# MPEGGroup/mpeg-pcc-tmc2

Hardware: AMD Instinct MI355X
Metric: encoder patch+image-gen frames/sec, longdress_vox10 32-frame GOF (higher is better)
Workload: dtype int32/f64

## Files before the change

### mpeg-pcc-tmc2_amd/csrc/attributes.hip

```cpp
#include <algorithm>
#include <cmath>

#include "color_transfer.h"
#include "internal.h"
#include "wave.h"
#include "patch_border_filter.h"

namespace tmc2 {
namespace {

__device__ __forceinline__ void toCanvasB( const PlaceDev& p, int u, int v, int& x, int& y ) {
  if ( p.orient == 0 ) {
    x = u + p.u0 * 16;
    y = v + p.v0 * 16;
  } else {
    x = v + p.u0 * 16;
    y = u + p.v0 * 16;
  }
}

__device__ __forceinline__ int normalCoord( const PlaceDev& p, int depth ) {
  return p.mode == 0 ? depth + p.d1 : max( 0, p.d1 - depth );
}

// ... 115 lines not shown
  reinterpret_cast<uchar4*>( outRgb4 )[t] = combinedColor( reinterpret_cast<const uchar4*>( fwdRgb4 )[t], c );
}

__device__ __forceinline__ CtColor ctColorOf( const uint8_t* __restrict__ rgb4, uint32_t i ) {
  const uchar4 c = reinterpret_cast<const uchar4*>( rgb4 )[i];
  return CtColor{c.x, c.y, c.z};
}
__device__ __forceinline__ void ctStore( uint8_t* __restrict__ rgb4, uint32_t i, const CtColor& c ) {
  reinterpret_cast<uchar4*>( rgb4 )[i] = make_uchar4( uint8_t( c.c0 ), uint8_t( c.c1 ), uint8_t( c.c2 ), 0 );
}
__global__ __launch_bounds__( 256 ) void forwardColorRulesKernel( const uint32_t* __restrict__ idx, const uint32_t* __restrict__ dist, int stride,
                                                                   const uint32_t* __restrict__ easy, const uint8_t* __restrict__ srcRgb4,
                                                                   uint32_t m, CtRules p, uint8_t* __restrict__ fwdRgb4 ) {
  const uint32_t t = blockIdx.x * blockDim.x + threadIdx.x;
  if ( t >= m ) return;
  if ( easy && easy[t] != 0xFFFFFFFFu ) {
    reinterpret_cast<uchar4*>( fwdRgb4 )[t] = reinterpret_cast<const uchar4*>( srcRgb4 )[easy[t]];
    return;
  }
  const uint32_t* id = idx + size_t( t ) * stride;
  const uint32_t* ds = dist + size_t( t ) * stride;
  ctStore( fwdRgb4, t, ctForward( p, p.kFwd, [ds]( int i ) { return ds[i]; }, [id, srcRgb4]( int i ) { return ctColorOf( srcRgb4, id[i] ); } ) );
}

template <bool FILL>
__global__ __launch_bounds__( 256 ) void backwardVoteRulesKernel( const uint32_t* __restrict__ idx, const uint32_t* __restrict__ dist, int stride,
                                                                   uint32_t n, int kBwd, double geoBwd, uint32_t* __restrict__ count,
                                                                   const uint32_t* __restrict__ offset, uint2* __restrict__ entries ) {
  const uint32_t s = blockIdx.x * blockDim.x + threadIdx.x;
  if ( s >= n ) return;
  for ( int r = 0; r < kBwd; ++r ) {
    const uint32_t d = dist[size_t( s ) * stride + r];
    if ( !( double( d ) <= geoBwd ) ) continue;
    const uint32_t t = idx[size_t( s ) * stride + r], slot = atomicAdd( &count[t], 1u );
    if ( FILL ) entries[offset[t] + slot] = make_uint2( d, s * uint32_t( kBwd ) + uint32_t( r ) );
  }
}

__global__ __launch_bounds__( 256 ) void combineColorRulesKernel( const uint32_t* __restrict__ count, const uint32_t* __restrict__ offset,
                                                                   uint2* __restrict__ entries, const uint8_t* __restrict__ srcRgb4,
                                                                   const uint8_t* __restrict__ fwdRgb4, uint32_t m, CtRules p, double rTarget,
                                                                   double rSource, uint8_t* __restrict__ outRgb4, uint32_t* __restrict__ error ) {
  const uint32_t t = blockIdx.x * blockDim.x + threadIdx.x;
  if ( t >= m ) return;
  const int     n   = int( count[t] );
  const CtColor fwd = ctColorOf( fwdRgb4, t );
  if ( n == 0 || p.lossless ) {
    ctStore( outRgb4, t, fwd );
    return;
  }
  uint2* e = entries + offset[t];
  if ( !orderCandidates( e, n ) ) *error = 1;
  const uint32_t kBwd = uint32_t( p.kBwd );
  ctStore( outRgb4, t,
           ctBackward( p, n, [e]( int i ) { return e[i].x; }, [e, srcRgb4, kBwd]( int i ) { return ctColorOf( srcRgb4, e[i].y / kBwd ); }, fwd,
                       rTarget, rSource ) );
}

__global__ __launch_bounds__( 256 ) void attributeScatterKernel( const uint8_t* __restrict__ rgb4,
                                                                  const uint32_t* __restrict__ pointToPixel, uint32_t m,
                                                                  int W, int H, uint8_t* __restrict__ attr ) {
  const uint32_t i = blockIdx.x * blockDim.x + threadIdx.x;
  if ( i >= m ) return;
  const uint32_t pp = pointToPixel[i];
  const size_t   px = size_t( pixelY( pp ) ) * W + pixelX( pp ), plane = size_t( W ) * H;
  const uchar4   c  = reinterpret_cast<const uchar4*>( rgb4 )[i];
  const bool     layer1 = pixelLayer( pp ), hasD1 = pixelHasD1( pp );
  if ( !layer1 ) {
    attr[px] = c.x, attr[plane + px] = c.y, attr[2 * plane + px] = c.z;
    if ( !hasD1 ) attr[3 * plane + px] = c.x, attr[4 * plane + px] = c.y, attr[5 * plane + px] = c.z;
  } else {
    attr[3 * plane + px] = c.x, attr[4 * plane + px] = c.y, attr[5 * plane + px] = c.z;
  }
}

__global__ __launch_bounds__( 256 ) void upsampleOccupancyKernel( const uint8_t* __restrict__ occVideo, int W, int H, int prec,
                                                                   uint8_t* __restrict__ occ ) {
  const size_t c = size_t( blockIdx.x ) * blockDim.x + threadIdx.x;
  if ( c >= size_t( W ) * H ) return;
  occ[c] = occVideo[size_t( ( c / W ) / prec ) * ( W / prec ) + ( c % W ) / prec];
}

__device__ __forceinline__ int mean4w( int p1, int w1, int p2, int w2, int p3, int w3, int p4, int w4 ) {
  return ( p1 * w1 + p2 * w2 + p3 * w3 + p4 * w4 ) / ( w1 + w2 + w3 + w4 );
}

__device__ __forceinline__ void pushPullMipPixel( int i, const uint8_t* img, const uint8_t* occ, int W, int H, uint8_t* mip,
                                                  uint8_t* mipOcc, int w, int h, int p0 = 0, int p1 = 6 ) {
  const int  x = i % w, y = i / w, X = 2 * x, Y = 2 * y;
  const bool i2 = X + 1 < W, i3 = Y + 1 < H;
  const int  w1 = occ[size_t( Y ) * W + X] ? 255 : 0;
  const int  w2 = ( i2 && occ[size_t( Y ) * W + X + 1] ) ? 255 : 0;
  const int  w3 = ( i3 && occ[size_t( Y + 1 ) * W + X] ) ? 255 : 0;
  const int  w4 = ( i2 && i3 && occ[size_t( Y + 1 ) * W + X + 1] ) ? 255 : 0;
  const bool any = ( w1 + w2 + w3 + w4 ) > 0;
  mipOcc[i]      = any ? 1 : 0;
  for ( int p = p0; p < p1; ++p ) {
    const uint8_t* s = img + size_t( p ) * W * H;
    uint8_t        v = 0;
    if ( any ) {
      const int v1 = s[size_t( Y ) * W + X], v2 = i2 ? s[size_t( Y ) * W + X + 1] : 0;
      const int v3 = i3 ? s[size_t( Y + 1 ) * W + X] : 0, v4 = ( i2 && i3 ) ? s[size_t( Y + 1 ) * W + X + 1] : 0;
      v            = uint8_t( mean4w( v1, w1, v2, w2, v3, w3, v4, w4 ) );
    }
    mip[size_t( p ) * w * h + i] = v;
  }
}
__global__ __launch_bounds__( 256 ) void pushPullMipKernel( const uint8_t* __restrict__ img, const uint8_t* __restrict__ occ, int W,
                                                             int H, uint8_t* __restrict__ mip, uint8_t* __restrict__ mipOcc, int w,
                                                             int h ) {
  const int i = blockIdx.x * blockDim.x + threadIdx.x;
  if ( i < w * h ) pushPullMipPixel( i, img, occ, W, H, mip, mipOcc, w, h );
}

__device__ __forceinline__ void pushPullFillPixel( int i, uint8_t* img, const uint8_t* occ, int W, int H, const uint8_t* mip, int w,
                                                   int h, int p0 = 0, int p1 = 6 ) {
  if ( occ[i] ) return;
  const int  X = i % W, Y = i / W, x = X >> 1, y = Y >> 1;
  const int  dx = ( X & 1 ) ? 1 : -1, dy = ( Y & 1 ) ? 1 : -1;
  const bool hx = dx < 0 ? x > 0 : x < w - 1, hy = dy < 0 ? y > 0 : y < h - 1;
  for ( int p = p0; p < p1; ++p ) {
    const uint8_t* m  = mip + size_t( p ) * w * h;
    const int      v  = m[size_t( y ) * w + x];
    const int      vx = hx ? m[size_t( y ) * w + x + dx] : 0;
    const int      vy = hy ? m[size_t( y + dy ) * w + x] : 0;
    const int      vd = ( hx && hy ) ? m[size_t( y + dy ) * w + x + dx] : 0;
    img[size_t( p ) * W * H + i] = uint8_t( mean4w( v, 144, vx, hx ? 48 : 0, vy, hy ? 48 : 0, vd, ( hx && hy ) ? 16 : 0 ) );
  }
}
__global__ __launch_bounds__( 256 ) void pushPullFillKernel( uint8_t* __restrict__ img, const uint8_t* __restrict__ occ, int W, int H,
                                                              const uint8_t* __restrict__ mip, int w, int h ) {
  const int i = blockIdx.x * blockDim.x + threadIdx.x;
  if ( i < W * H ) pushPullFillPixel( i, img, occ, W, H, mip, w, h );
}

__device__ __forceinline__ void pushPullBlurPixel( int i, const uint8_t* src, uint8_t* dst, const uint8_t* occ, int W, int H, int p0 = 0,
                                                   int p1 = 6 ) {
  if ( occ[i] ) return;
  const int x = i % W, y = i / W;
  const int x1 = x > 0 ? x - 1 : x, y1 = y > 0 ? y - 1 : y, x2 = x < W - 1 ? x + 1 : x, y2 = y < H - 1 ? y + 1 : y;
  for ( int p = p0; p < p1; ++p ) {
    const uint8_t* s   = src + size_t( p ) * W * H;
    const int      sum = s[size_t( y1 ) * W + x1] + s[size_t( y1 ) * W + x2] + s[size_t( y2 ) * W + x1] + s[size_t( y2 ) * W + x2] +
                    s[size_t( y ) * W + x1] + s[size_t( y ) * W + x2] + s[size_t( y1 ) * W + x] + s[size_t( y2 ) * W + x];
    dst[size_t( p ) * W * H + i] = uint8_t( ( sum + 4 ) >> 3 );
  }
}
__global__ __launch_bounds__( 256 ) void pushPullBlurKernel( const uint8_t* __restrict__ src, uint8_t* __restrict__ dst,
                                                              const uint8_t* __restrict__ occ, int W, int H ) {
  const int i = blockIdx.x * blockDim.x + threadIdx.x;
  if ( i < W * H ) pushPullBlurPixel( i, src, dst, occ, W, H );
}

constexpr int kPushPullTile = 96, kPushPullSpan = 128, kPushPullMaxIters = ( kPushPullSpan - kPushPullTile ) / 2;
__global__ __launch_bounds__( 1024 ) void pushPullFillBlurKernel( uint8_t* __restrict__ img, const uint8_t* __restrict__ occ, int W,
                                                                   int H, const uint8_t* __restrict__ mip, int w, int h, int iters,
                                                                   int tilesX ) {
  __shared__ uint8_t sOcc[kPushPullSpan * kPushPullSpan];
  __shared__ uint8_t sBuf[2][kPushPullSpan * kPushPullSpan];
  const int      X0 = ( blockIdx.x % tilesX ) * kPushPullTile, Y0 = ( blockIdx.x / tilesX ) * kPushPullTile;
  const int      RX0 = max( X0 - iters, 0 ), RY0 = max( Y0 - iters, 0 );
  const int      RW = min( X0 + kPushPullTile + iters, W ) - RX0, RH = min( Y0 + kPushPullTile + iters, H ) - RY0;
  uint8_t*       plane = img + size_t( blockIdx.y ) * W * H;
  const uint8_t* m     = mip + size_t( blockIdx.y ) * w * h;
  for ( int i = threadIdx.x; i < kPushPullSpan * RH; i += 1024 ) {
    const int rx = i & ( kPushPullSpan - 1 ), ry = i >> 7;
    if ( rx >= RW ) continue;
    const int     X = RX0 + rx, Y = RY0 + ry;
    const size_t  g = size_t( Y ) * W + X;
    const uint8_t o = occ[g];
    uint8_t       v;
    if ( o ) {
      v = plane[g];
    } else {
      const int  x = X >> 1, y = Y >> 1, dx = ( X & 1 ) ? 1 : -1, dy = ( Y & 1 ) ? 1 : -1;
      const bool hx = dx < 0 ? x > 0 : x < w - 1, hy = dy < 0 ? y > 0 : y < h - 1;
      const int  c  = m[size_t( y ) * w + x];
      const int  vx = hx ? m[size_t( y ) * w + x + dx] : 0;
      const int  vy = hy ? m[size_t( y + dy ) * w + x] : 0;
      const int  vd = ( hx && hy ) ? m[size_t( y + dy ) * w + x + dx] : 0;
      v             = uint8_t( mean4w( c, 144, vx, hx ? 48 : 0, vy, hy ? 48 : 0, vd, ( hx && hy ) ? 16 : 0 ) );
    }
    sOcc[i]    = o;
    sBuf[0][i] = v;
    sBuf[1][i] = v;
  }
  __syncthreads();
  int cur = 0;
  for ( int it = 0; it < iters; ++it ) {
    const uint8_t* src = sBuf[cur];
    uint8_t*       dst = sBuf[cur ^ 1];
    for ( int i = threadIdx.x; i < kPushPullSpan * RH; i += 1024 ) {
      const int rx = i & ( kPushPullSpan - 1 ), ry = i >> 7;
      if ( rx >= RW || sOcc[i] ) continue;
      const int l = rx > 0 ? -1 : 0, r = rx < RW - 1 ? 1 : 0;
      const int u = ry > 0 ? -kPushPullSpan : 0, d = ry < RH - 1 ? kPushPullSpan : 0;
      const int sum = src[i + u + l] + src[i + u + r] + src[i + d + l] + src[i + d + r] + src[i + l] + src[i + r] + src[i + u] +
                      src[i + d];
      dst[i] = uint8_t( ( sum + 4 ) >> 3 );
    }
    __syncthreads();
    cur ^= 1;
  }
  const uint8_t* res = sBuf[cur];
  for ( int i = threadIdx.x; i < kPushPullSpan * RH; i += 1024 ) {
    const int rx = i & ( kPushPullSpan - 1 ), ry = i >> 7;
    const int X = RX0 + rx, Y = RY0 + ry;
    if ( rx >= RW || sOcc[i] || X < X0 || X >= X0 + kPushPullTile || Y < Y0 || Y >= Y0 + kPushPullTile ) continue;
    plane[size_t( Y ) * W + X] = res[i];
  }
}

constexpr int kPushPullSmall  = 160 * 160;
constexpr int kPushPullLevels = 16;
struct PushPullLevels {
  int      count;
  int      first;
  int      w[kPushPullLevels], h[kPushPullLevels];
  uint8_t *img[kPushPullLevels], *tmp[kPushPullLevels], *occ[kPushPullLevels];
};
__global__ __launch_bounds__( 1024 ) void pushPullCoarseLevelsKernel( PushPullLevels L ) {
  const int p0 = int( blockIdx.x ), p1 = p0 + 1;
  for ( int l = L.first + 1; l < L.count; ++l ) {
    const int cnt = L.w[l] * L.h[l];
    for ( int i = threadIdx.x; i < cnt; i += blockDim.x )
      pushPullMipPixel( i, L.img[l - 1], L.occ[l - 1], L.w[l - 1], L.h[l - 1], L.img[l], L.occ[l], L.w[l], L.h[l], p0, p1 );
    __syncthreads();
  }
  int iters = 4;
  for ( int l = L.count - 1; l > L.first; --l ) {
    const int fw = L.w[l - 1], fh = L.h[l - 1], cnt = fw * fh;
    uint8_t * img = L.img[l - 1], *tmp = L.tmp[l - 1];
    const uint8_t* occ = L.occ[l - 1];
    for ( int i = threadIdx.x; i < cnt; i += blockDim.x ) pushPullFillPixel( i, img, occ, fw, fh, L.img[l], L.w[l], L.h[l], p0, p1 );
    __syncthreads();
    for ( int i = threadIdx.x; i < cnt; i += blockDim.x ) tmp[size_t( p0 ) * cnt + i] = img[size_t( p0 ) * cnt + i];
    __syncthreads();
    uint8_t *src = img, *dst = tmp;
    for ( int it = 0; it < iters; ++it ) {
      for ( int i = threadIdx.x; i < cnt; i += blockDim.x ) pushPullBlurPixel( i, src, dst, occ, fw, fh, p0, p1 );
      __syncthreads();
      uint8_t* t = src;
      src        = dst;
      dst        = t;
    }
    if ( src != img ) {
      L.img[l - 1] = src;
      L.tmp[l - 1] = img;
    }
    iters = min( iters + 1, 16 );
  }
}

__global__ __launch_bounds__( 256 ) void attributeGroupDilateKernel( const uint8_t* __restrict__ occ, int W, int H,
                                                                      uint8_t* __restrict__ attr ) {
  const size_t c = size_t( blockIdx.x ) * blockDim.x + threadIdx.x, plane = size_t( W ) * H;
  if ( c >= plane || occ[c] ) return;
#pragma unroll
  for ( int k = 0; k < 3; ++k ) {
    const uint32_t a = attr[k * plane + c], b = attr[( 3 + k ) * plane + c];
    const uint8_t  v = uint8_t( ( a + b + 1 ) >> 1 );
    attr[k * plane + c] = attr[( 3 + k ) * plane + c] = v;
  }
}

}

static int transferColorsRules( tmc2_ctx* ctx, const TreeDev& srcTree, const Pt* d_srcPts, const uint8_t* d_srcRgb4, uint32_t n,
                                const TreeDev& tgtTree, const Pt* d_tgtPts, uint32_t M, uint8_t* d_outRgb4, uint32_t* d_error,
                                const CtRules& p ) {
  hipStream_t      s = ctx->stream;
  const dim3       blk( 256 );
  const int        wf = knnWidth( p.kFwd ), wb = knnWidth( p.kBwd );
  DevBuf<uint32_t> d_idxF, d_distF, d_easyF, d_idxB, d_distB, d_count, d_offset, d_cursor;
  DevBuf<uint2>    d_entries;
  DevBuf<uint8_t>  d_fwd;
  TMC2_TRY( d_idxF.alloc( size_t( M ) * wf ) );
  TMC2_TRY( d_distF.alloc( size_t( M ) * wf ) );
  TMC2_TRY( d_idxB.alloc( size_t( n ) * wb ) );
  TMC2_TRY( d_distB.alloc( size_t( n ) * wb ) );
  TMC2_TRY( d_count.alloc( M ) );
  TMC2_TRY( d_offset.alloc( M ) );
  TMC2_TRY( d_cursor.alloc( M ) );
  TMC2_TRY( d_entries.alloc( size_t( n ) * p.kBwd ) );
  TMC2_TRY( d_fwd.alloc( size_t( M ) * 4 ) );
  if ( p.skipFwd ) {
    TMC2_TRY( d_easyF.alloc( M ) );
    TMC2_TRY( launchKnnSplit( ctx, srcTree, d_tgtPts, M, wf, d_easyF.p, d_idxF.p, d_distF.p, "knn_recon_in_source", false, p.kFwd ) );
  } else {
    TMC2_TRY( launchKnnTree( ctx, srcTree, d_tgtPts, M, wf, d_idxF.p, d_distF.p, "knn_recon_in_source", p.kFwd ) );
  }
  if ( p.kBwd == 1 )
    TMC2_TRY( launchKnnSplit( ctx, tgtTree, d_srcPts, n, 1, d_idxB.p, d_idxB.p, d_distB.p, "knn_source_in_recon" ) );
  else
    TMC2_TRY( launchKnnTree( ctx, tgtTree, d_srcPts, n, wb, d_idxB.p, d_distB.p, "knn_source_in_recon", p.kBwd ) );
  StageScope stage( ctx, "transfer_colors" );
  TMC2_TRY( fillRegions( ctx, {{d_count.p, size_t( M ) * 4, 0}, {d_cursor.p, size_t( M ) * 4, 0}, {d_error, 4, 0}} ) );
  const dim3 grdM( ( M + 255 ) / 256 ), grdN( ( n + 255 ) / 256 );
  hipLaunchKernelGGL( forwardColorRulesKernel, grdM, blk, 0, s, d_idxF.p, d_distF.p, wf, p.skipFwd ? d_easyF.p : (const uint32_t*)nullptr,
                      d_srcRgb4, M, p, d_fwd.p );
  hipLaunchKernelGGL( backwardVoteRulesKernel<false>, grdN, blk, 0, s, d_idxB.p, d_distB.p, wb, n, p.kBwd, p.geoBwd, d_count.p, d_offset.p,
                      d_entries.p );
  TMC2_TRY( exclusiveScanU32( ctx, d_count.p, d_offset.p, M, nullptr ) );
  hipLaunchKernelGGL( backwardVoteRulesKernel<true>, grdN, blk, 0, s, d_idxB.p, d_distB.p, wb, n, p.kBwd, p.geoBwd, d_cursor.p, d_offset.p,
                      d_entries.p );
  hipLaunchKernelGGL( combineColorRulesKernel, grdM, blk, 0, s, d_count.p, d_offset.p, d_entries.p, d_srcRgb4, d_fwd.p, M, p,
                      1.0 / double( M ), 1.0 / double( n ), d_outRgb4, d_error );
  TMC2_HIP( hipGetLastError() );
  return TMC2_OK;
}

int transferColorsDevice( tmc2_ctx* ctx, const TreeDev& srcTree, const Pt* d_srcPts, const uint8_t* d_srcRgb4, uint32_t n,
                          const TreeDev& tgtTree, const Pt* d_tgtPts, uint32_t M, uint8_t* d_outRgb4, uint32_t* d_error,
                          const tmc2_color_transfer_params* params = nullptr ) {
  const auto forced = ctxOption( ctx, "COLOR_TRANSFER_RULES" );
  if ( params && ( !ctIsDefault( *params ) || ( forced && ( *forced )[0] == '1' ) ) )
    return transferColorsRules( ctx, srcTree, d_srcPts, d_srcRgb4, n, tgtTree, d_tgtPts, M, d_outRgb4, d_error, ctRules( *params ) );
  hipStream_t      s = ctx->stream;
  const dim3       blk( 256 );
  DevBuf<uint32_t> d_idx8, d_dist8, d_idx1, d_dist1, d_count, d_offset, d_cursor;
  DevBuf<uint2>    d_entries;
  DevBuf<uint8_t>  d_fwd;
  TMC2_TRY( d_idx8.alloc( size_t( M ) * 8 ) );
  TMC2_TRY( d_dist8.alloc( size_t( M ) * 8 ) );
  TMC2_TRY( d_idx1.alloc( n ) );
  TMC2_TRY( d_dist1.alloc( n ) );
  TMC2_TRY( d_count.alloc( M ) );
  TMC2_TRY( d_offset.alloc( M ) );
  TMC2_TRY( d_cursor.alloc( M ) );
  TMC2_TRY( d_entries.alloc( n ) );
  TMC2_TRY( d_fwd.alloc( size_t( M ) * 4 ) );
  DevBuf<uint32_t> d_easy8;
  TMC2_TRY( d_easy8.alloc( M ) );
  TMC2_TRY( launchKnnSplit( ctx, srcTree, d_tgtPts, M, 8, d_easy8.p, d_idx8.p, d_dist8.p, "knn8_recon_in_source" ) );
  TMC2_TRY( launchKnnSplit( ctx, tgtTree, d_srcPts, n, 1, d_idx1.p, d_idx1.p, d_dist1.p, "knn1_source_in_recon" ) );
  StageScope stage( ctx, "transfer_colors" );
  TMC2_TRY( fillRegions( ctx, {{d_count.p, size_t( M ) * 4, 0}, {d_cursor.p, size_t( M ) * 4, 0}, {d_error, 4, 0}} ) );
  const dim3 grdM( ( M + 255 ) / 256 ), grdN( ( n + 255 ) / 256 );
  hipLaunchKernelGGL( forwardColorKernel, grdM, blk, 0, s, d_idx8.p, d_dist8.p, d_easy8.p, d_srcRgb4, M, d_fwd.p );
  hipLaunchKernelGGL( backwardVoteKernel<false>, grdN, blk, 0, s, d_idx1.p, d_dist1.p, n, d_count.p, d_offset.p, d_entries.p );
  TMC2_TRY( exclusiveScanU32( ctx, d_count.p, d_offset.p, M, nullptr ) );
  hipLaunchKernelGGL( backwardVoteKernel<true>, grdN, blk, 0, s, d_idx1.p, d_dist1.p, n, d_cursor.p, d_offset.p, d_entries.p );
  hipLaunchKernelGGL( combineColorKernel, grdM, blk, 0, s, d_count.p, d_offset.p, d_entries.p, d_srcRgb4, d_fwd.p, M,
                      d_outRgb4, d_error );
  TMC2_HIP( hipGetLastError() );
  return TMC2_OK;
}

int reconstructPointCloud( tmc2_frame* f, const PbfParams* pbfParams ) {
  if ( !f->haveGeometryImages ) {
    setError( "generatePointCloud: geometry images missing" );
    return TMC2_E_STATE;
  }
  if ( pbfParams ) {
    if ( const char* what = pbfRefusal( f->occPrecision, *pbfParams, long( f->patches.size() ) ) ) {
      setError( "generatePointCloud (patch border filtering): unsupported %s", what );
      return TMC2_E_UNSUPPORTED;
    }
  }
  const bool keepAttributeImages = f->haveAttributeImages && ( pbfParams || f->havePbf );
  f->canvasesChanged();
  f->haveAttributeImages = keepAttributeImages;
  if ( pbfParams ) TMC2_TRY( patchBorderFilterDevice( f, *pbfParams ) );
  PbfMapsDev pbf;
  if ( pbfParams ) pbf = PbfMapsDev{f->d_pbfOffset.p, f->pbfOcc, f->pbfFlag, f->pbfBorderWidth, nullptr};
  tmc2_ctx*    ctx = f->ctx;
  hipStream_t  s   = ctx->stream;
  const int    W = f->canvasW, H = f->canvasH, prec = f->occPrecision;
  const dim3   blk( 256 );
  const uint32_t tiles = f->tileCount;
  StageScope       stage( ctx, "reconstruct" );
  DevBuf<uint32_t> d_tileCount, d_tileOffset, d_small;
  TMC2_TRY( d_tileCount.alloc( std::max( tiles, 1u ) ) );
  TMC2_TRY( d_tileOffset.alloc( std::max( tiles, 1u ) ) );
  TMC2_TRY( d_small.alloc( 8 ) );
  uint32_t M = 0;
  if ( tiles ) {
    if ( pbfParams )
      hipLaunchKernelGGL( ( reconTileKernel<false, true> ), dim3( tiles ), blk, 0, s, f->d_place.p, f->d_tilePatch.p, f->d_occVideo.p,
                          f->d_blockToPatch.p, f->d_geo.p, W, H, prec, d_tileCount.p, (const uint32_t*)nullptr, (Pt*)nullptr,
                          (uint32_t*)nullptr, pbf );
    else
      hipLaunchKernelGGL( reconTileKernel<false>, dim3( tiles ), blk, 0, s, f->d_place.p, f->d_tilePatch.p, f->d_occVideo.p,
                          f->d_blockToPatch.p, f->d_geo.p, W, H, prec, d_tileCount.p, (const uint32_t*)nullptr, (Pt*)nullptr,
                          (uint32_t*)nullptr, PbfMapsDev() );
    volatile uint32_t* answer = ctx->answerLine( tmc2_ctx::kAnswerRecon );
    TMC2_TRY( exclusiveScanU32( ctx, d_tileCount.p, d_tileOffset.p, tiles, d_small.p, ScanAnswer{answer, nullptr, 0} ) );
    TMC2_HIP( hipStreamSynchronize( s ) );
    M = answer[0];
  }
  if ( M == 0 && pbfParams ) {
    stage.end();
    f->reconCount         = 0;
    f->haveReconstruction = true;
    f->haveBoundaryTypes  = true;
    return TMC2_OK;
  }
  if ( M == 0 ) {
    setError( "generatePointCloud: empty reconstruction" );
    return TMC2_E_STATE;
  }
  TMC2_TRY( f->d_recon.alloc( M ) );
  TMC2_TRY( f->d_pointToPixel.alloc( M ) );
  if ( pbfParams ) {
    TMC2_TRY( f->d_boundaryType.alloc( M ) );
    TMC2_TRY( f->d_pbfBoundary.alloc( M ) );
    pbf.btype = f->d_boundaryType.p;
    hipLaunchKernelGGL( ( reconTileKernel<true, true> ), dim3( tiles ), blk, 0, s, f->d_place.p, f->d_tilePatch.p, f->d_occVideo.p,
                        f->d_blockToPatch.p, f->d_geo.p, W, H, prec, d_tileCount.p, d_tileOffset.p, f->d_recon.p, f->d_pointToPixel.p,
                        pbf );
    TMC2_HIP( hipMemcpyAsync( f->d_pbfBoundary.p, f->d_boundaryType.p, M, hipMemcpyDeviceToDevice, s ) );
  } else {
    hipLaunchKernelGGL( reconTileKernel<true>, dim3( tiles ), blk, 0, s, f->d_place.p, f->d_tilePatch.p, f->d_occVideo.p,
                        f->d_blockToPatch.p, f->d_geo.p, W, H, prec, d_tileCount.p, d_tileOffset.p, f->d_recon.p,
                        f->d_pointToPixel.p, PbfMapsDev() );
  }
  stage.end();
  f->reconCount = M;
  TMC2_TRY( buildKdTreePlaced( ctx, f->d_recon.p, M, nullptr, "kdtree_build_recon", f->reconTree ) );
  f->haveReconstruction = true;
  f->haveBoundaryTypes  = pbfParams != nullptr;
  return TMC2_OK;
}

static int reconstructionSize( tmc2_frame* f, uint32_t* M ) {
  tmc2_ctx*      ctx   = f->ctx;
  const uint32_t tiles = f->tileCount;
  *M                   = 0;
  if ( !tiles ) return TMC2_OK;
  DevBuf<uint32_t> d_tileCount, d_tileOffset, d_small;
  TMC2_TRY( d_tileCount.alloc( tiles ) );
  TMC2_TRY( d_tileOffset.alloc( tiles ) );
  TMC2_TRY( d_small.alloc( 8 ) );
  hipLaunchKernelGGL( reconTileKernel<false>, dim3( tiles ), dim3( 256 ), 0, ctx->stream, f->d_place.p, f->d_tilePatch.p, f->d_occVideo.p,
                      f->d_blockToPatch.p, f->d_geo.p, f->canvasW, f->canvasH, f->occPrecision, d_tileCount.p, (const uint32_t*)nullptr,
                      (Pt*)nullptr, (uint32_t*)nullptr, PbfMapsDev() );
  volatile uint32_t* answer = ctx->answerLine( tmc2_ctx::kAnswerRecon );
  TMC2_TRY( exclusiveScanU32( ctx, d_tileCount.p, d_tileOffset.p, tiles, d_small.p, ScanAnswer{answer, nullptr, 0} ) );
  TMC2_HIP( hipStreamSynchronize( ctx->stream ) );
  *M = answer[0];
  return TMC2_OK;
}

int generateAttributeImages( tmc2_frame* f, const tmc2_color_transfer_params* params ) {
  if ( !f->haveGeometryImages ) {
    setError( "generateAttributeImages: geometry images missing" );
    return TMC2_E_STATE;
  }
  if ( f->d_rgb.count == 0 ) {
    setError( "generateAttributeImages: the frame has no colours" );
    return TMC2_E_STATE;
  }
  if ( params ) {
    TMC2_TRY( checkColorTransferParams( "generateAttributeImages", params, f->n, 0 ) );
    if ( params->numNeighborsColorTransferBwd > 1 ) {
      uint32_t size = 0;
      TMC2_TRY( reconstructionSize( f, &size ) );
      if ( size ) TMC2_TRY( checkColorTransferParams( "generateAttributeImages", params, f->n, size ) );
    }
  }
  TMC2_TRY( f->ensureTree() );
  TMC2_TRY( reconstructPointCloud( f ) );
  tmc2_ctx*    ctx = f->ctx;
  hipStream_t  s   = ctx->stream;
  const int    W = f->canvasW, H = f->canvasH, prec = f->occPrecision;
  const size_t area = size_t( W ) * H;
  const dim3   blk( 256 );
  const uint32_t n = uint32_t( f->n ), M = uint32_t( f->reconCount );
  DevBuf<uint32_t> d_small;
  TMC2_TRY( d_small.alloc( 8 ) );
  TMC2_TRY( f->d_reconRgb.alloc( size_t( M ) * 4 ) );
  const dim3 grdM( ( M + 255 ) / 256 );
  volatile uint32_t* h_err = ctx->answerLine( tmc2_ctx::kAnswerAttrError );
  TMC2_TRY( transferColorsDevice( ctx, f->tree.view( QueryBox::Tight ), f->d_pts.p, f->d_rgb.p, n, f->reconTree.view( QueryBox::Tight ),
                                  f->d_recon.p, M, f->d_reconRgb.p, const_cast<uint32_t*>( h_err ), params ) );
  StageScope      stage( ctx, "attribute_images" );
  DevBuf<uint8_t> d_occ;
  TMC2_TRY( d_occ.alloc( area ) );
  TMC2_TRY( f->d_attr.alloc( 6 * area ) );
  TMC2_HIP( hipMemsetAsync( f->d_attr.p, 0, 6 * area, s ) );
  hipLaunchKernelGGL( upsampleOccupancyKernel, dim3( uint32_t( ( area + 255 ) / 256 ) ), blk, 0, s, f->d_occVideo.p, W, H, prec,
                      d_occ.p );
  hipLaunchKernelGGL( attributeScatterKernel, grdM, blk, 0, s, f->d_reconRgb.p, f->d_pointToPixel.p, M, W, H, f->d_attr.p );
  struct Level {
    int      w, h;
    uint8_t *img, *tmp, *occ;
  };
  std::vector<Level> lv;
  lv.push_back( Level{W, H, f->d_attr.p, nullptr, d_occ.p} );
  size_t pyramidBytes = 6 * area;
  {
    int w = W, h = H;
    for ( ;; ) {
      w = ( w + 1 ) >> 1;
      h = ( h + 1 ) >> 1;
      lv.push_back( Level{w, h, nullptr, nullptr, nullptr} );
      pyramidBytes += size_t( w ) * h * ( 6 + 6 + 1 );
      if ( w <= 4 || h <= 4 ) break;
    }
  }
  DevBuf<uint8_t> d_pyr;
  TMC2_TRY( d_pyr.alloc( pyramidBytes + 64 * lv.size() ) );
  {
    uint8_t* p = d_pyr.p;
    lv[0].tmp  = p;
    p += 6 * area;
    for ( size_t l = 1; l < lv.size(); ++l ) {
      const size_t a = size_t( lv[l].w ) * lv[l].h;
      lv[l].img = p, p += 6 * a;
      lv[l].tmp = p, p += 6 * a;
      lv[l].occ = p, p += ( a + 15 ) & ~size_t( 15 );
    }
  }
  size_t firstSmall = lv.size();
  if ( lv.size() <= size_t( kPushPullLevels ) )
    for ( size_t l = 1; l < lv.size(); ++l )
      if ( lv[l].w * lv[l].h <= kPushPullSmall ) {
        firstSmall = l;
        break;
      }
  for ( size_t l = 1; l < lv.size() && l <= firstSmall; ++l ) {
    const int cnt = lv[l].w * lv[l].h;
    hipLaunchKernelGGL( pushPullMipKernel, dim3( ( cnt + 255 ) / 256 ), blk, 0, s, lv[l - 1].img, lv[l - 1].occ, lv[l - 1].w,
                        lv[l - 1].h, lv[l].img, lv[l].occ, lv[l].w, lv[l].h );
  }
  int iters = 4;
  if ( firstSmall + 1 < lv.size() ) {
    PushPullLevels L;
    L.count = int( lv.size() ), L.first = int( firstSmall );
    for ( size_t l = 0; l < lv.size(); ++l ) L.w[l] = lv[l].w, L.h[l] = lv[l].h, L.img[l] = lv[l].img, L.tmp[l] = lv[l].tmp, L.occ[l] = lv[l].occ;
    hipLaunchKernelGGL( pushPullCoarseLevelsKernel, dim3( 6 ), dim3( 1024 ), 0, s, L );
    for ( size_t l = lv.size() - 1; l > firstSmall; --l ) {
      if ( iters & 1 ) std::swap( lv[l - 1].img, lv[l - 1].tmp );
      iters = std::min( iters + 1, 16 );
    }
  }
  for ( size_t l = std::min( firstSmall, lv.size() - 1 ); l >= 1; --l ) {
    Level&    fine = lv[l - 1];
    const int cnt  = fine.w * fine.h;
    const dim3 grd( ( cnt + 255 ) / 256 );
    if ( iters <= kPushPullMaxIters ) {
      const int tilesX = ( fine.w + kPushPullTile - 1 ) / kPushPullTile, tilesY = ( fine.h + kPushPullTile - 1 ) / kPushPullTile;
      hipLaunchKernelGGL( pushPullFillBlurKernel, dim3( tilesX * tilesY, 6 ), dim3( 1024 ), 0, s, fine.img, fine.occ, fine.w, fine.h,
                          lv[l].img, lv[l].w, lv[l].h, iters, tilesX );
      iters = std::min( iters + 1, 16 );
      continue;
    }
    hipLaunchKernelGGL( pushPullFillKernel, grd, blk, 0, s, fine.img, fine.occ, fine.w, fine.h, lv[l].img, lv[l].w, lv[l].h );
    TMC2_HIP( hipMemcpyAsync( fine.tmp, fine.img, size_t( 6 ) * cnt, hipMemcpyDeviceToDevice, s ) );
    uint8_t *src = fine.img, *dst = fine.tmp;
    for ( int it = 0; it < iters; ++it ) {
      hipLaunchKernelGGL( pushPullBlurKernel, grd, blk, 0, s, src, dst, fine.occ, fine.w, fine.h );
      std::swap( src, dst );
    }
    if ( src != fine.img ) {
      if ( l - 1 == 0 )
        TMC2_HIP( hipMemcpyAsync( fine.img, src, size_t( 6 ) * cnt, hipMemcpyDeviceToDevice, s ) );
      else
        std::swap( fine.img, fine.tmp );
    }
    iters = std::min( iters + 1, 16 );
  }
  hipLaunchKernelGGL( attributeGroupDilateKernel, dim3( uint32_t( ( area + 255 ) / 256 ) ), blk, 0, s, d_occ.p, W, H, f->d_attr.p );
  stage.end();
  TMC2_HIP( hipStreamSynchronize( s ) );
  TMC2_HIP( hipGetLastError() );
  const uint32_t err = *h_err;
  if ( err ) {
    setError( "transferColors: a backward candidate list hit std::sort's depth limit (heapsort fallback of libstdc++ "
              "introsort is not reproduced)" );
    return TMC2_E_UNSUPPORTED;
  }
  f->haveAttributeImages = true;
  return TMC2_OK;
}

}

extern "C" {

int tmc2_transfer_colors_ex( tmc2_ctx* ctx, const int16_t* srcXyz, const uint8_t* srcRgb, uint64_t n, const int16_t* tgtXyz, uint64_t m,
                             const tmc2_color_transfer_params* params, uint8_t* tgtRgb ) {
  using namespace tmc2;
  if ( !ctx || !srcXyz || !srcRgb || !tgtXyz || !tgtRgb || n < 1 || m < 1 || n > 0x3FFFFFFull || m > 0x7FFFFFF0ull ) {
    setError( "transfer_colors: invalid argument" );
    return TMC2_E_INVALID;
  }
  TMC2_TRY( checkColorTransferParams( "transfer_colors", params, n, m ) );
  ApiScope    scope( ctx );
  hipStream_t s = ctx->stream;
  struct Side {
    DevBuf<Pt> pts;
    DeviceTree tree;
  } S, T;
  auto upload = [&]( Side& sd, const int16_t* xyz, uint64_t cnt ) -> int {
    std::vector<Pt> pts( cnt );
    for ( uint64_t i = 0; i < cnt; ++i ) pts[i] = Pt{xyz[3 * i], xyz[3 * i + 1], xyz[3 * i + 2], 0};
    TMC2_TRY( sd.pts.alloc( cnt ) );
    TMC2_HIP( hipMemcpyAsync( sd.pts.p, pts.data(), cnt * sizeof( Pt ), hipMemcpyHostToDevice, s ) );
    TMC2_HIP( hipStreamSynchronize( s ) );
    return buildKdTreeDevice( ctx, sd.pts.p, cnt, sd.tree );
  };
  TMC2_TRY( upload( S, srcXyz, n ) );
  TMC2_TRY( upload( T, tgtXyz, m ) );
  std::vector<uint8_t> c4( 4 * n );
  for ( uint64_t i = 0; i < n; ++i ) c4[4 * i] = srcRgb[3 * i], c4[4 * i + 1] = srcRgb[3 * i + 1], c4[4 * i + 2] = srcRgb[3 * i + 2], c4[4 * i + 3] = 0;
  DevBuf<uint8_t>  d_rgb, d_out;
  DevBuf<uint32_t> d_err;
  TMC2_TRY( d_rgb.alloc( 4 * n ) );
  TMC2_TRY( d_out.alloc( 4 * m ) );
  TMC2_TRY( d_err.alloc( 1 ) );
  TMC2_HIP( hipMemcpyAsync( d_rgb.p, c4.data(), 4 * n, hipMemcpyHostToDevice, s ) );
  TMC2_TRY( transferColorsDevice( ctx, S.tree.view( QueryBox::Any ), S.pts.p, d_rgb.p, uint32_t( n ), T.tree.view( QueryBox::Any ), T.pts.p,
                                  uint32_t( m ), d_out.p, d_err.p, params ) );
  std::vector<uint8_t> o4( 4 * m );
  uint32_t             err = 0;
  TMC2_HIP( hipMemcpyAsync( o4.data(), d_out.p, 4 * m, hipMemcpyDeviceToHost, s ) );
  TMC2_HIP( hipMemcpyAsync( &err, d_err.p, 4, hipMemcpyDeviceToHost, s ) );
  TMC2_HIP( hipStreamSynchronize( s ) );
  if ( err ) {
    setError( "transferColors: a backward candidate list hit std::sort's depth limit (not reproduced)" );
    return TMC2_E_UNSUPPORTED;
  }
  for ( uint64_t i = 0; i < m; ++i ) tgtRgb[3 * i] = o4[4 * i], tgtRgb[3 * i + 1] = o4[4 * i + 1], tgtRgb[3 * i + 2] = o4[4 * i + 2];
  return TMC2_OK;
}

int tmc2_transfer_colors( tmc2_ctx* ctx, const int16_t* srcXyz, const uint8_t* srcRgb, uint64_t n, const int16_t* tgtXyz,
                          uint64_t m, uint8_t* tgtRgb ) {
  if ( !ctx || !srcXyz || !srcRgb || !tgtXyz || !tgtRgb || n < 8 || m < 1 ) {
    tmc2::setError( "transfer_colors: invalid argument (the source needs at least 8 points)" );
    return TMC2_E_INVALID;
  }
  tmc2_color_transfer_params ctc;
  tmc2::ctDefault( ctc );
  return tmc2_transfer_colors_ex( ctx, srcXyz, srcRgb, n, tgtXyz, m, &ctc, tgtRgb );
}

int tmc2_codec_generate_point_cloud( tmc2_frame* f ) {
  if ( !f ) return TMC2_E_INVALID;
  tmc2::ApiScope scope( f->ctx );
  return tmc2::reconstructPointCloud( f );
}

int tmc2_encoder_generate_attribute_images_ex( tmc2_frame* f, const tmc2_color_transfer_params* params ) {
  if ( !f ) return TMC2_E_INVALID;
  if ( !params ) {
    tmc2::setError( "generateAttributeImages: the colour-transfer parameters are NULL" );
    return TMC2_E_INVALID;
  }
  tmc2::ApiScope scope( f->ctx );
  return tmc2::generateAttributeImages( f, params );
}

int tmc2_encoder_generate_attribute_images( tmc2_frame* f ) {
  if ( !f ) return TMC2_E_INVALID;
  tmc2_color_transfer_params ctc;
  tmc2::ctDefault( ctc );
  return tmc2_encoder_generate_attribute_images_ex( f, &ctc );
}

int64_t tmc2_frame_recon_count( tmc2_frame* f ) { return ( f && f->haveReconstruction ) ? int64_t( f->reconCount ) : 0; }

int tmc2_frame_get_reconstruction( tmc2_frame* f, int16_t* xyz, uint8_t* rgb, uint32_t* pointToPixel ) {
  if ( !f || !f->haveReconstruction ) {
    tmc2::setError( "get_reconstruction: not generated" );
    return TMC2_E_STATE;
  }
  if ( rgb && ( !f->haveAttributeImages || f->havePbf ) ) {
    tmc2::setError( "get_reconstruction: no transferred colours (tmc2_encoder_generate_attribute_images produces them)" );
    return TMC2_E_STATE;
  }
  tmc2::ApiScope scope( f->ctx );
  hipStream_t    s = f->ctx->stream;
  const size_t   M = f->reconCount;
  if ( M == 0 ) return TMC2_OK;
  std::vector<tmc2::Pt>  pts( M );
  std::vector<uint8_t>   c4( rgb ? 4 * M : 0 );
  std::vector<uint32_t>  pp( M );
  TMC2_HIP( hipMemcpyAsync( pts.data(), f->d_recon.p, M * sizeof( tmc2::Pt ), hipMemcpyDeviceToHost, s ) );
  if ( rgb ) TMC2_HIP( hipMemcpyAsync( c4.data(), f->d_reconRgb.p, 4 * M, hipMemcpyDeviceToHost, s ) );
  TMC2_HIP( hipMemcpyAsync( pp.data(), f->d_pointToPixel.p, 4 * M, hipMemcpyDeviceToHost, s ) );
  TMC2_HIP( hipStreamSynchronize( s ) );
  for ( size_t i = 0; i < M; ++i ) {
    if ( xyz ) xyz[3 * i] = pts[i].x, xyz[3 * i + 1] = pts[i].y, xyz[3 * i + 2] = pts[i].z;
    if ( rgb ) rgb[3 * i] = c4[4 * i], rgb[3 * i + 1] = c4[4 * i + 1], rgb[3 * i + 2] = c4[4 * i + 2];
    if ( pointToPixel )
      pointToPixel[3 * i] = tmc2::pixelX( pp[i] ), pointToPixel[3 * i + 1] = tmc2::pixelY( pp[i] ), pointToPixel[3 * i + 2] = tmc2::pixelLayer( pp[i] );
  }
  return TMC2_OK;
}

int tmc2_frame_device_attribute( tmc2_frame* f, void** attribute ) {
  if ( !f || !attribute || !f->haveAttributeImages ) return TMC2_E_STATE;
  *attribute = f->d_attr.p;
  return TMC2_OK;
// ... 14 lines not shown
```

Measured before the change: 219.4.

## Pack push-pull blur into SWAR words and keep coarse pyramid in LDS

Rewrites the tiled fill+blur kernel to process four 8-bit pixels per 32-bit word with SWAR arithmetic and per-thread vertical strips that reuse rows held in registers. It narrows the blur region each iteration, shrinking the halo, and exits early for tiles with no holes. The coarse-level kernel now builds the whole small pyramid (mip, fill, blur) in dynamic shared memory instead of global buffers, raising the LDS limit when needed. This cuts global traffic and per-pixel instruction count, at the cost of tricky edge masking, a different fill formula that clamps neighbours instead of reweighting them, and a large LDS footprint that may limit occupancy.

```diff
diff --git a/mpeg-pcc-tmc2_amd/csrc/attributes.hip b/mpeg-pcc-tmc2_amd/csrc/attributes.hip
--- a/mpeg-pcc-tmc2_amd/csrc/attributes.hip
+++ b/mpeg-pcc-tmc2_amd/csrc/attributes.hip
@@ -291,103 +291,261 @@
   if ( i < W * H ) pushPullBlurPixel( i, src, dst, occ, W, H );
 }
 
+struct PushPullEdge {
+  bool     first;
+  bool     last3;
+  uint32_t after;
+};
+__device__ __forceinline__ PushPullEdge pushPullEdge( int wx, int w ) {
+  const bool last = wx == ( ( w - 1 ) >> 2 );
+  const int  b    = ( w - 1 ) & 3;
+  return PushPullEdge{wx == 0, last && b == 3, last && b < 3 ? 0xFF00u << ( 8 * b ) : 0u};
+}
+struct PushPullRow {
+  uint32_t lo, hi, e;
+};
+__device__ __forceinline__ PushPullRow pushPullRowTerms( uint32_t l, uint32_t c, uint32_t r, const PushPullEdge& E ) {
+  constexpr uint32_t kF = 0x00FF00FFu;
+  const uint32_t     cp = ( c & ~E.after ) | ( ( c << 8 ) & E.after );
+  const uint32_t     lb = E.first ? c & 0xFFu : l >> 24, rb = E.last3 ? c >> 24 : r & 0xFFu;
+  return PushPullRow{cp & kF, ( cp >> 8 ) & kF, lb | ( rb << 16 )};
+}
+template <int R>
+__device__ __forceinline__ void pushPullBlurStrip( const uint32_t* __restrict__ src, uint32_t* __restrict__ dst,
+                                                   const uint32_t* __restrict__ occ, int pitch, int rows, int wx, int y0, int y1,
+                                                   const PushPullEdge& E ) {
+  constexpr uint32_t kF = 0x00FF00FFu;
+  const int          oLast = ( rows - 1 ) * pitch + wx;
+  int                o = y0 * pitch + wx;
+  const uint32_t*    s = src + max( o - pitch, wx );
+  PushPullRow        up = pushPullRowTerms( s[-1], s[0], s[1], E );
+  s                     = src + o;
+  uint32_t    cw  = s[0];
+  PushPullRow mid = pushPullRowTerms( s[-1], cw, s[1], E );
+  for ( int y = y0; y < y1; y += R ) {
+    uint32_t l[R], c[R], r[R], m[R];
+    int      at[R];
+#pragma unroll
+    for ( int k = 0; k < R; ++k ) {
+      at[k]               = min( o + k * pitch, oLast );
+      const uint32_t* n   = src + min( o + ( k + 1 ) * pitch, oLast );
+      l[k] = n[-1], c[k] = n[0], r[k] = n[1], m[k] = occ[at[k]];
+    }
+#pragma unroll
+    for ( int k = 0; k < R; ++k ) asm volatile( "" : "+v"( m[k] ) );
+#pragma unroll
+    for ( int k = 0; k < R; ++k ) {
+      const PushPullRow dn  = pushPullRowTerms( l[k], c[k], r[k], E );
+      const uint32_t    vlo = up.lo + mid.lo + dn.lo, vhi = up.hi + mid.hi + dn.hi, ve = up.e + mid.e + dn.e, t = vlo + vhi;
+      const uint32_t slo = t + ( ( vhi << 16 ) | ( ve & 0xFFFFu ) ), shi = t + ( ( vlo >> 16 ) | ( ve & 0xFFFF0000u ) );
+      const uint32_t lo = ( ( slo - mid.lo + 0x00040004u ) >> 3 ) & kF, hi = ( ( shi - mid.hi + 0x00040004u ) >> 3 ) & kF;
+      if ( y + k < y1 ) dst[at[k]] = ( cw & m[k] ) | ( ( lo | ( hi << 8 ) ) & ~m[k] );
+      up = mid, mid = dn, cw = c[k];
+    }
+    o += R * pitch;
+  }
+}
+
+__device__ __forceinline__ uint32_t pushPullFillValue( const uint8_t* m, int pitch, int w, int h, int X, int Y ) {
+  const int      x = X >> 1, y = Y >> 1;
+  const int      xn = ( X & 1 ) ? min( x + 1, w - 1 ) : max( x - 1, 0 ), yn = ( Y & 1 ) ? min( y + 1, h - 1 ) : max( y - 1, 0 );
+  const uint8_t *r0 = m + size_t( y ) * pitch, *r1 = m + size_t( yn ) * pitch;
+  return ( 9u * r0[x] + 3u * r0[xn] + 3u * r1[x] + r1[xn] ) >> 4;
+}
+
+__device__ __forceinline__ uint32_t pushPullLoad4( const uint8_t* p ) {
+  uint32_t v;
+  __builtin_memcpy( &v, p, 4 );
+  return v;
+}
+
 constexpr int kPushPullTile = 96, kPushPullSpan = 128, kPushPullMaxIters = ( kPushPullSpan - kPushPullTile ) / 2;
-__global__ __launch_bounds__( 1024 ) void pushPullFillBlurKernel( uint8_t* __restrict__ img, const uint8_t* __restrict__ occ, int W,
-                                                                   int H, const uint8_t* __restrict__ mip, int w, int h, int iters,
-                                                                   int tilesX ) {
-  __shared__ uint8_t sOcc[kPushPullSpan * kPushPullSpan];
-  __shared__ uint8_t sBuf[2][kPushPullSpan * kPushPullSpan];
+constexpr int kPushPullPitch = kPushPullSpan / 4, kPushPullWords = kPushPullPitch * kPushPullSpan;
+constexpr int kPushPullThreads = 512, kPushPullStrips = kPushPullThreads / kPushPullPitch;
+static_assert( kPushPullThreads % kPushPullPitch == 0 && kPushPullThreads <= 1024, "whole strips of word columns" );
+__global__ __launch_bounds__( kPushPullThreads ) void pushPullFillBlurKernel( uint8_t* __restrict__ img, const uint8_t* __restrict__ occ,
+                                                                               int W, int H, const uint8_t* __restrict__ mip, int w, int h,
+                                                                               int iters, int tilesX ) {
+  __shared__ uint32_t sOcc[kPushPullWords];
+  __shared__ uint32_t sBuf[2 * kPushPullWords + 2];
   const int      X0 = ( blockIdx.x % tilesX ) * kPushPullTile, Y0 = ( blockIdx.x / tilesX ) * kPushPullTile;
   const int      RX0 = max( X0 - iters, 0 ), RY0 = max( Y0 - iters, 0 );
   const int      RW = min( X0 + kPushPullTile + iters, W ) - RX0, RH = min( Y0 + kPushPullTile + iters, H ) - RY0;
+  const int      CX0 = X0 - RX0, CX1 = min( X0 + kPushPullTile, W ) - RX0, CY0 = Y0 - RY0, CY1 = min( Y0 + kPushPullTile, H ) - RY0;
   uint8_t*       plane = img + size_t( blockIdx.y ) * W * H;
   const uint8_t* m     = mip + size_t( blockIdx.y ) * w * h;
-  for ( int i = threadIdx.x; i < kPushPullSpan * RH; i += 1024 ) {
-    const int rx = i & ( kPushPullSpan - 1 ), ry = i >> 7;
-    if ( rx >= RW ) continue;
-    const int     X = RX0 + rx, Y = RY0 + ry;
-    const size_t  g = size_t( Y ) * W + X;
-    const uint8_t o = occ[g];
-    uint8_t       v;
-    if ( o ) {
-      v = plane[g];
-    } else {
-      const int  x = X >> 1, y = Y >> 1, dx = ( X & 1 ) ? 1 : -1, dy = ( Y & 1 ) ? 1 : -1;
-      const bool hx = dx < 0 ? x > 0 : x < w - 1, hy = dy < 0 ? y > 0 : y < h - 1;
-      const int  c  = m[size_t( y ) * w + x];
-      const int  vx = hx ? m[size_t( y ) * w + x + dx] : 0;
-      const int  vy = hy ? m[size_t( y + dy ) * w + x] : 0;
-      const int  vd = ( hx && hy ) ? m[size_t( y + dy ) * w + x + dx] : 0;
-      v             = uint8_t( mean4w( c, 144, vx, hx ? 48 : 0, vy, hy ? 48 : 0, vd, ( hx && hy ) ? 16 : 0 ) );
-    }
-    sOcc[i]    = o;
-    sBuf[0][i] = v;
-    sBuf[1][i] = v;
-  }
-  __syncthreads();
-  int cur = 0;
+  const int      wx = threadIdx.x & ( kPushPullPitch - 1 ), strip = threadIdx.x / kPushPullPitch;
+  const int      rx0 = 4 * wx, XW = RX0 + rx0, mb = w >= 4 ? min( max( ( XW >> 1 ) - 1, 0 ), w - 4 ) : 0;
+  const uint32_t coreX = ( rx0 >= CX0 && rx0 < CX1 ? 0xFFu : 0u ) | ( rx0 + 1 >= CX0 && rx0 + 1 < CX1 ? 0xFF00u : 0u ) |
+                         ( rx0 + 2 >= CX0 && rx0 + 2 < CX1 ? 0xFF0000u : 0u ) | ( rx0 + 3 >= CX0 && rx0 + 3 < CX1 ? 0xFF000000u : 0u );
+  int            hole  = 0;
+  if ( rx0 + 3 < RW && w >= 4 ) {
+#pragma unroll 4
+    for ( int ry = strip; ry < RH; ry += kPushPullStrips ) {
+      const int      Y = RY0 + ry, y = Y >> 1, yn = ( Y & 1 ) ? min( y + 1, h - 1 ) : max( y - 1, 0 );
+      const size_t   g  = size_t( Y ) * W + XW;
+      const uint32_t o4 = pushPullLoad4( occ + g ), p4 = pushPullLoad4( plane + g );
+      const uint32_t r0 = pushPullLoad4( m + size_t( y ) * w + mb ), r1 = pushPullLoad4( m + size_t( yn ) * w + mb );
+      const uint32_t nz = ( ( ( o4 & 0x7F7F7F7Fu ) + 0x7F7F7F7Fu ) | o4 ) & 0x80808080u, msk = ( nz >> 7 ) * 0xFFu;
+      uint32_t       fill = 0;
+#pragma unroll
+      for ( int j = 0; j < 4; ++j ) {
+        const int      X = XW + j, x = X >> 1, xn = ( X & 1 ) ? min( x + 1, w - 1 ) : max( x - 1, 0 ), sx = 8 * ( x - mb ), sn = 8 * ( xn - mb );
+        fill |= ( ( 9u * ( ( r0 >> sx ) & 0xFFu ) + 3u * ( ( r0 >> sn ) & 0xFFu ) + 3u * ( ( r1 >> sx ) & 0xFFu ) + ( ( r1 >> sn ) & 0xFFu ) ) >> 4 ) << ( 8 * j );
+      }
+      const uint32_t pix = ( p4 & msk ) | ( fill & ~msk );
+      const int      i   = ry * kPushPullPitch + wx;
+      hole |= int( ( ~msk & coreX ) != 0 && ry >= CY0 && ry < CY1 );
+      sOcc[i] = msk, sBuf[1 + i] = pix, sBuf[1 + kPushPullWords + i] = pix;
+    }
+  } else {
+    for ( int ry = strip; ry < RH; ry += kPushPullStrips ) {
+      const int Y = RY0 + ry, i = ry * kPushPullPitch + wx;
+      uint32_t  pix = 0, msk = 0;
+#pragma unroll
+      for ( int j = 0; j < 4; ++j ) {
+        const int rx = rx0 + j, X = RX0 + rx;
+        uint32_t  v = 0, o = 0xFFu;
+        if ( rx < RW ) {
+          const size_t g = size_t( Y ) * W + X;
+          o              = occ[g] ? 0xFFu : 0u;
+          v              = o ? uint32_t( plane[g] ) : pushPullFillValue( m, w, w, h, X, Y );
+          hole |= int( !o && rx >= CX0 && rx < CX1 && ry >= CY0 && ry < CY1 );
+        }
+        pix |= v << ( 8 * j ), msk |= o << ( 8 * j );
+      }
+      sOcc[i] = msk, sBuf[1 + i] = pix, sBuf[1 + kPushPullWords + i] = pix;
+    }
+  }
+  if ( !__syncthreads_or( hole ) ) return;
+  const PushPullEdge edge = pushPullEdge( wx, RW );
+  int            cur = 0;
   for ( int it = 0; it < iters; ++it ) {
-    const uint8_t* src = sBuf[cur];
-    uint8_t*       dst = sBuf[cur ^ 1];
-    for ( int i = threadIdx.x; i < kPushPullSpan * RH; i += 1024 ) {
-      const int rx = i & ( kPushPullSpan - 1 ), ry = i >> 7;
-      if ( rx >= RW || sOcc[i] ) continue;
-      const int l = rx > 0 ? -1 : 0, r = rx < RW - 1 ? 1 : 0;
-      const int u = ry > 0 ? -kPushPullSpan : 0, d = ry < RH - 1 ? kPushPullSpan : 0;
-      const int sum = src[i + u + l] + src[i + u + r] + src[i + d + l] + src[i + d + r] + src[i + l] + src[i + r] + src[i + u] +
-                      src[i + d];
-      dst[i] = uint8_t( ( sum + 4 ) >> 3 );
-    }
+    const int g  = iters - 1 - it;
+    const int xa = max( X0 - g, 0 ) - RX0, xb = min( X0 + kPushPullTile + g, W ) - RX0;
+    const int ya = max( Y0 - g, 0 ) - RY0, yb = min( Y0 + kPushPullTile + g, H ) - RY0;
+    const int per = ( yb - ya + kPushPullStrips - 1 ) / kPushPullStrips, y0 = ya + strip * per, y1 = min( y0 + per, yb );
+    if ( wx >= ( xa >> 2 ) && wx <= ( ( xb - 1 ) >> 2 ) && y0 < y1 )
+      pushPullBlurStrip<4>( sBuf + 1 + cur * kPushPullWords, sBuf + 1 + ( cur ^ 1 ) * kPushPullWords, sOcc, kPushPullPitch, RH, wx, y0, y1,
+                            edge );
     __syncthreads();
     cur ^= 1;
   }
-  const uint8_t* res = sBuf[cur];
-  for ( int i = threadIdx.x; i < kPushPullSpan * RH; i += 1024 ) {
-    const int rx = i & ( kPushPullSpan - 1 ), ry = i >> 7;
-    const int X = RX0 + rx, Y = RY0 + ry;
-    if ( rx >= RW || sOcc[i] || X < X0 || X >= X0 + kPushPullTile || Y < Y0 || Y >= Y0 + kPushPullTile ) continue;
-    plane[size_t( Y ) * W + X] = res[i];
+  const uint32_t* res = sBuf + 1 + cur * kPushPullWords;
+  for ( int i = kPushPullPitch * CY0 + threadIdx.x; i < kPushPullPitch * CY1; i += kPushPullThreads ) {
+    const int      cx = i & ( kPushPullPitch - 1 ), ry = i / kPushPullPitch;
+    const uint32_t v = res[i], o = sOcc[i];
+#pragma unroll
+    for ( int j = 0; j < 4; ++j ) {
+      const int rx = 4 * cx + j;
+      if ( rx >= CX0 && rx < CX1 && !( ( o >> ( 8 * j ) ) & 0xFFu ) ) plane[size_t( RY0 + ry ) * W + RX0 + rx] = uint8_t( v >> ( 8 * j ) );
+    }
   }
 }
 
 constexpr int kPushPullSmall  = 160 * 160;
 constexpr int kPushPullLevels = 16;
 struct PushPullLevels {
-  int      count;
-  int      first;
-  int      w[kPushPullLevels], h[kPushPullLevels];
-  uint8_t *img[kPushPullLevels], *tmp[kPushPullLevels], *occ[kPushPullLevels];
+  int            count;
+  int            first;
+  int            w[kPushPullLevels], h[kPushPullLevels];
+  const uint8_t *img, *occ;
+  uint8_t*       out;
 };
+__host__ __device__ inline int pushPullLevelWords( int w, int h ) { return 3 * ( ( w + 3 ) >> 2 ) * h + 2; }
 __global__ __launch_bounds__( 1024 ) void pushPullCoarseLevelsKernel( PushPullLevels L ) {
-  const int p0 = int( blockIdx.x ), p1 = p0 + 1;
+  extern __shared__ uint32_t sPyr[];
+  const int plane = int( blockIdx.x ), tid = int( threadIdx.x );
+  int       w = L.w[L.first], h = L.h[L.first], pw = ( w + 3 ) >> 2, n = pw * h, base = 0;
+  {
+    const uint8_t* src = L.img + size_t( plane ) * w * h;
+    uint32_t *     img = sPyr + base + 1, *occ = sPyr + base + 2 + 2 * n;
+    for ( int i = tid; i < n; i += 1024 ) {
+      const int wx = i % pw, y = i / pw;
+      uint32_t  pix = 0, msk = 0;
+#pragma unroll
+      for ( int j = 0; j < 4; ++j ) {
+        const int x = 4 * wx + j;
+        uint32_t  v = 0, o = 0xFFu;
+        if ( x < w ) {
+          const size_t g = size_t( y ) * w + x;
+          o = L.occ[g] ? 0xFFu : 0u, v = src[g];
+        }
+        pix |= v << ( 8 * j ), msk |= o << ( 8 * j );
+      }
+      img[i] = pix, occ[i] = msk;
+    }
+  }
+  __syncthreads();
   for ( int l = L.first + 1; l < L.count; ++l ) {
-    const int cnt = L.w[l] * L.h[l];
-    for ( int i = threadIdx.x; i < cnt; i += blockDim.x )
-      pushPullMipPixel( i, L.img[l - 1], L.occ[l - 1], L.w[l - 1], L.h[l - 1], L.img[l], L.occ[l], L.w[l], L.h[l], p0, p1 );
+    const int      W = w, H = h, fp = 4 * pw;
+    const uint8_t *fimg = reinterpret_cast<const uint8_t*>( sPyr + base + 1 ), *focc = reinterpret_cast<const uint8_t*>( sPyr + base + 2 + 2 * n );
+    base += 3 * n + 2;
+    w = L.w[l], h = L.h[l], pw = ( w + 3 ) >> 2, n = pw * h;
+    uint32_t *img = sPyr + base + 1, *occ = sPyr + base + 2 + 2 * n;
+    for ( int i = tid; i < n; i += 1024 ) {
+      const int wx = i % pw, y = i / pw, Y = 2 * y;
+      uint32_t  pix = 0, msk = 0;
+#pragma unroll
+      for ( int j = 0; j < 4; ++j ) {
+        const int x = 4 * wx + j, X = 2 * x;
+        uint32_t  v = 0, o = 0xFFu;
+        if ( x < w ) {
+          const bool i2 = X + 1 < W, i3 = Y + 1 < H;
+          const int  a = Y * fp + X;
+          const bool o1 = focc[a], o2 = i2 && focc[a + 1], o3 = i3 && focc[a + fp], o4 = i2 && i3 && focc[a + fp + 1];
+          const int  cnt = int( o1 ) + int( o2 ) + int( o3 ) + int( o4 );
+          const int  sum = ( o1 ? fimg[a] : 0 ) + ( o2 ? fimg[a + 1] : 0 ) + ( o3 ? fimg[a + fp] : 0 ) + ( o4 ? fimg[a + fp + 1] : 0 );
+          o              = cnt ? 0xFFu : 0u;
+          v              = cnt == 3 ? uint32_t( sum ) / 3u : uint32_t( sum ) >> ( cnt >> 1 );
+        }
+        pix |= v << ( 8 * j ), msk |= o << ( 8 * j );
+      }
+      img[i] = pix, occ[i] = msk;
+    }
     __syncthreads();
   }
-  int iters = 4;
+  int iters = 4, inTmp = 0;
   for ( int l = L.count - 1; l > L.first; --l ) {
-    const int fw = L.w[l - 1], fh = L.h[l - 1], cnt = fw * fh;
-    uint8_t * img = L.img[l - 1], *tmp = L.tmp[l - 1];
-    const uint8_t* occ = L.occ[l - 1];
-    for ( int i = threadIdx.x; i < cnt; i += blockDim.x ) pushPullFillPixel( i, img, occ, fw, fh, L.img[l], L.w[l], L.h[l], p0, p1 );
+    const int      cw = w, ch = h, cp = 4 * pw;
+    const uint8_t* m = reinterpret_cast<const uint8_t*>( sPyr + base + 1 + ( inTmp ? n : 0 ) );
+    w = L.w[l - 1], h = L.h[l - 1], pw = ( w + 3 ) >> 2, n = pw * h;
+    base -= 3 * n + 2;
+    uint32_t *      img = sPyr + base + 1, *tmp = img + n;
+    const uint32_t* occ = sPyr + base + 2 + 2 * n;
+    for ( int i = tid; i < n; i += 1024 ) {
+      const int      wx = i % pw, y = i / pw;
+      const uint32_t msk = occ[i];
+      uint32_t       pix = img[i];
+#pragma unroll
+      for ( int j = 0; j < 4; ++j )
+        if ( !( ( msk >> ( 8 * j ) ) & 0xFFu ) ) pix = ( pix & ~( 0xFFu << ( 8 * j ) ) ) | ( pushPullFillValue( m, cp, cw, ch, 4 * wx + j, y ) << ( 8 * j ) );
+      img[i] = pix, tmp[i] = pix;
+    }
     __syncthreads();
-    for ( int i = threadIdx.x; i < cnt; i += blockDim.x ) tmp[size_t( p0 ) * cnt + i] = img[size_t( p0 ) * cnt + i];
-    __syncthreads();
-    uint8_t *src = img, *dst = tmp;
+    const int per = ( h + max( 1024 / pw, 1 ) - 1 ) / max( 1024 / pw, 1 ), strips = ( h + per - 1 ) / per;
     for ( int it = 0; it < iters; ++it ) {
-      for ( int i = threadIdx.x; i < cnt; i += blockDim.x ) pushPullBlurPixel( i, src, dst, occ, fw, fh, p0, p1 );
+      const uint32_t* src = ( it & 1 ) ? tmp : img;
+      uint32_t*       dst = ( it & 1 ) ? img : tmp;
+      for ( int i = tid; i < pw * strips; i += 1024 ) {
+        const int wx = i % pw, y0 = ( i / pw ) * per;
+        pushPullBlurStrip<2>( src, dst, occ, pw, h, wx, y0, min( y0 + per, h ), pushPullEdge( wx, w ) );
+      }
       __syncthreads();
-      uint8_t* t = src;
-      src        = dst;
-      dst        = t;
-    }
-    if ( src != img ) {
-      L.img[l - 1] = src;
-      L.tmp[l - 1] = img;
-    }
+    }
+    inTmp = iters & 1;
     iters = min( iters + 1, 16 );
+  }
+  {
+    const uint32_t* res = sPyr + base + 1 + ( inTmp ? n : 0 );
+    uint8_t*        out = L.out + size_t( plane ) * w * h;
+    for ( int i = tid; i < n; i += 1024 ) {
+      const int      wx = i % pw, y = i / pw;
+      const uint32_t v = res[i];
+#pragma unroll
+      for ( int j = 0; j < 4; ++j )
+        if ( 4 * wx + j < w ) out[size_t( y ) * w + 4 * wx + j] = uint8_t( v >> ( 8 * j ) );
+    }
   }
 }
 
@@ -651,11 +809,14 @@
       lv[l].occ = p, p += ( a + 15 ) & ~size_t( 15 );
     }
   }
-  size_t firstSmall = lv.size();
+  size_t                firstSmall = lv.size(), coarseLds = 0;
+  constexpr size_t      kCoarseLdsMax = 160 * 1024 - 64;
+  std::vector<size_t>   ldsFrom( lv.size() + 1, 0 );
+  for ( size_t l = lv.size(); l-- > 1; ) ldsFrom[l] = ldsFrom[l + 1] + sizeof( uint32_t ) * size_t( pushPullLevelWords( lv[l].w, lv[l].h ) );
   if ( lv.size() <= size_t( kPushPullLevels ) )
     for ( size_t l = 1; l < lv.size(); ++l )
-      if ( lv[l].w * lv[l].h <= kPushPullSmall ) {
-        firstSmall = l;
+      if ( lv[l].w * lv[l].h <= kPushPullSmall && ldsFrom[l] <= kCoarseLdsMax ) {
+        firstSmall = l, coarseLds = ldsFrom[l];
         break;
       }
   for ( size_t l = 1; l < lv.size() && l <= firstSmall; ++l ) {
@@ -667,12 +828,16 @@
   if ( firstSmall + 1 < lv.size() ) {
     PushPullLevels L;
     L.count = int( lv.size() ), L.first = int( firstSmall );
-    for ( size_t l = 0; l < lv.size(); ++l ) L.w[l] = lv[l].w, L.h[l] = lv[l].h, L.img[l] = lv[l].img, L.tmp[l] = lv[l].tmp, L.occ[l] = lv[l].occ;
-    hipLaunchKernelGGL( pushPullCoarseLevelsKernel, dim3( 6 ), dim3( 1024 ), 0, s, L );
+    for ( size_t l = 0; l < lv.size(); ++l ) L.w[l] = lv[l].w, L.h[l] = lv[l].h;
+    L.img = lv[firstSmall].img, L.occ = lv[firstSmall].occ;
     for ( size_t l = lv.size() - 1; l > firstSmall; --l ) {
       if ( iters & 1 ) std::swap( lv[l - 1].img, lv[l - 1].tmp );
       iters = std::min( iters + 1, 16 );
     }
+    L.out = lv[firstSmall].img;
+    if ( coarseLds > 48 * 1024 )
+      TMC2_TRY( allowLargeLds( reinterpret_cast<const void*>( pushPullCoarseLevelsKernel ), coarseLds, ctx->device ) );
+    hipLaunchKernelGGL( pushPullCoarseLevelsKernel, dim3( 6 ), dim3( 1024 ), coarseLds, s, L );
   }
   for ( size_t l = std::min( firstSmall, lv.size() - 1 ); l >= 1; --l ) {
     Level&    fine = lv[l - 1];
@@ -680,7 +845,7 @@
     const dim3 grd( ( cnt + 255 ) / 256 );
     if ( iters <= kPushPullMaxIters ) {
       const int tilesX = ( fine.w + kPushPullTile - 1 ) / kPushPullTile, tilesY = ( fine.h + kPushPullTile - 1 ) / kPushPullTile;
-      hipLaunchKernelGGL( pushPullFillBlurKernel, dim3( tilesX * tilesY, 6 ), dim3( 1024 ), 0, s, fine.img, fine.occ, fine.w, fine.h,
+      hipLaunchKernelGGL( pushPullFillBlurKernel, dim3( tilesX * tilesY, 6 ), dim3( kPushPullThreads ), 0, s, fine.img, fine.occ, fine.w, fine.h,
                           lv[l].img, lv[l].w, lv[l].h, iters, tilesX );
       iters = std::min( iters + 1, 16 );
       continue;
```

New measurement: 224.8, median of 6. 2.5% higher.
